# mmSir/SpatioTemporalEntropyModel

Hardware: AMD Instinct MI355X
Metric: frames/s (higher is better)
Workload: dtype f32; 1 GPU; configs[1]: SpatioTemporalPriorModel_Res(256,192) training step on mbt2018(192,192) latents, 16 septuplets x 7 frames x 256x256 per GPU, EMLoss, clip 1.0 + Adam 1e-4 / aux Adam 1e-3; per_gpu_batch=16, global_batch=16, parallelism=dp1, stream_priorities=latents=0,side=-1,compute=-1, stream_cu_masks=latents=block:160, plan_selectors=library defaults

## Files before the change

spatiotemporalentropymodel_amd/csrc/conv_f16x3.hip:

```cpp
#include <math.h>
#include <stdlib.h>

#include <type_traits>

#include "f16x3_tail.h"

namespace {

constexpr int XP = BN + 4;
constexpr int imax(int a, int b) { return a > b ? a : b; }
constexpr int lds_stages(int depth) { return depth == 3 ? 3 : 2; }
constexpr int lds_taps(int bm, int depth) { return imax(imax(lds_stages(depth) * NPL * (bm + BN) * 64, 6 * NPL * bm * 64 + NPL * BN * 64), bm * XP * 4); }
constexpr int lds_total(int bm, int depth) { return lds_taps(bm, depth) + 32 * 4; }

struct Fx3Phase {
    int ntaps, S;
    int dy0, dx0;
    int wofs;
    int cps, nsplit;
    int wsofs;
    int ooy, oox;
};

struct Fx3Args {
    const void *xp, *wp;
    const float *xq, *wq;
    float *yq;
    const float *bias, *beta;
    const void *gp;
    const float *gq;
    float *y;
    void *yp;
    int ldy;
    int B, H, W, C, N, OH, OW, stride, ntaps;
    int S;
    int xbytes, wbytes, gbytes;
    float beta_bound;
    int fuse;
    const float *z;
    int ldz, epi;
    float slope;
    float *ws;
    int *cnt;
    int nsplit, cps;
    int xpix;
    signed char dy[MAXTAP], dx[MAXTAP];
    int ptiles, btaps, OHf, OWf;
    Fx3Phase ph[4];
};

#define TAP_OFFSET(t) (tw_first + ((t) / tw_S) * tw_line + ((t) % tw_S) * tw_col)
#define TAP_WALK_NEXT()                                                                         \
    do {                                                                                        \
        const bool wrap_ = pf_t + 1 == tw_T, rowend_ = pf_ts + 1 == tw_S;                       \
        ++pf_q;                                                                                 \
        pf_to = wrap_ ? tw_first : pf_to + (rowend_ ? tw_line - (tw_S - 1) * tw_col : tw_col);  \
        pf_ts = (wrap_ || rowend_) ? 0 : pf_ts + 1;                                             \
        pf_t = wrap_ ? 0 : pf_t + 1;                                                            \
        pf_kc += wrap_ ? 1 : 0;                                                                 \
    } while (0)


__device__ inline int pi4(int x) { return (0x78 >> (2 * x)) & 3; }

typedef int rsrc4 __attribute__((ext_vector_type(4)));
__device__ inline rsrc4 dma_rsrc(const void *p, int bytes)
{
    const unsigned long long v = reinterpret_cast<unsigned long long>(p);
    return rsrc4{(int)(unsigned)v, (int)(unsigned)(v >> 32), bytes, 0x00020000};
}
__device__ inline void dma16(const rsrc4 r, unsigned lds_base, int voff, int soff)
{
    asm volatile("s_mov_b32 m0, %0\n\ts_nop 0\n\tbuffer_load_dwordx4 %1, %2, %3 offen lds" ::"s"(lds_base), "v"(voff), "s"(r), "s"(soff) : "memory");
}
#define DMA_WAIT_BARRIER(n) asm volatile("s_waitcnt vmcnt(%0)\n\ts_barrier" ::"n"(n) : "memory")
#define LDS_READS_DONE()                            \
    do {                                            \
        __builtin_amdgcn_sched_barrier(0);          \
        __builtin_amdgcn_s_waitcnt(0xC07F);         \
        __builtin_amdgcn_sched_barrier(0);          \
    } while (0)

template <int BM, int DEPTH, int MS>
__global__ __launch_bounds__(BM * 4) void conv_f16x3_kernel(const Fx3Args a)
{
    static_assert(DEPTH == 2 || DEPTH == 3, "two or three LDS stages");
    static_assert(MS == 32 || (MS == 16 && DEPTH == 3), "the 16-row MFMA shape exists for the three-stage loop");
    constexpr int NT = BM * 4;
    constexpr int A_PLANE = BM * 64, A_BUF = NPL * A_PLANE;
    constexpr int PL = NPL;
    constexpr int WPIECES = PL * BN * 4;
    static_assert(WPIECES % NT == 0, "every wavefront copies whole 1 KiB pieces of the weight chunk");
    constexpr int BP = WPIECES / NT;
    constexpr int NI = PL + BP;
    extern __shared__ __attribute__((aligned(16))) unsigned char smem[];
    constexpr int NST = lds_stages(DEPTH);
    unsigned char *As = smem;
    unsigned char *Bs = smem + NST * A_BUF;

    const int tid = threadIdx.x, lane = tid & 63, wave = tid >> 6;
    const int Mtot = a.B * a.OH * a.OW;
    int tile_m = blockIdx.x;
    {
        const int nb = gridDim.x, qq = nb >> 3, rr = nb & 7, xcd = tile_m & 7, idx = tile_m >> 3;
        if (nb >= 16) tile_m = (xcd < rr ? xcd * (qq + 1) : rr * (qq + 1) + (xcd - rr) * qq) + idx;
    }
    const int bm0 = tile_m * BM;
    const int nslab = a.C / KC, pixbytes = nslab * SLAB;

    const int srow = tid >> 2, scol = (tid & 3) ^ ((srow >> 2) & 3);
    int pb;
    unsigned pmask = 0;
    {
        const int m = bm0 + srow;
        const bool ok = m < Mtot;
        const int mm = ok ? m : 0;
        const int ohw = a.OH * a.OW, b = mm / ohw, rem = mm - b * ohw, qy = rem / a.OW, qx = rem - qy * a.OW;
        const int by = qy * a.stride, bx = qx * a.stride;
        pb = ((b * a.H + by) * a.W + bx) * pixbytes + scol * 16;
        for (int t = 0; t < a.ntaps; ++t) {
            const int iy = by + a.dy[t], ix = bx + a.dx[t];
            if (ok && iy >= 0 && iy < a.H && ix >= 0 && ix < a.W) pmask |= 1u << t;
        }
    }
    const int wv0 = tid * 16;
    const int nchunks = a.ntaps * nslab;
    const int q_last = nchunks - 1;
    __syncthreads();

    const rsrc4 rx = dma_rsrc(a.xp, a.xbytes), rw = dma_rsrc(a.wp, a.wbytes);
    const unsigned lds0 = (unsigned)(unsigned long long)(__attribute__((address_space(3))) unsigned char *)smem;
    const unsigned ldsw = __builtin_amdgcn_readfirstlane(lds0 + wave * 1024);
    auto dma_range = [&](int stage, int t, int tA, int kc, int q, int lo, int hi) {
        const int sA = kc * SLAB, sB = q * B_BUF;
        const int mk = __builtin_amdgcn_sbfe((int)pmask, (unsigned)t, 1u);
        const int off = ((pb + tA) & mk) | (OOR & ~mk);
        const unsigned la = ldsw + stage * A_BUF, lb = ldsw + NST * A_BUF + stage * B_BUF;
#pragma unroll
        for (int i = lo; i < hi; ++i) {
            if (i < PL)
                dma16(rx, la + i * A_PLANE, off + i * 64, sA);
            else
                dma16(rw, lb + (i - PL) * (NT * 16), wv0 + (i - PL) * (NT * 16), sB);
        }
    };
    auto dma = [&](int stage, int t, int tA, int kc, int q) { dma_range(stage, t, tA, kc, q, 0, NI); };

    const int wm0 = (wave >> 1) * 32, wn0 = (wave & 1) * 96;
    const int lr = lane & 31, lh = lane >> 5;
    const int sw = (lr >> 2) & 3;
    const int rdA = (wm0 + lr) * 64, rdB = (wn0 + lr) * 64;
    const int pk0 = ((0 + lh) ^ sw) << 4, pk1 = ((2 + lh) ^ sw) << 4;
    const int l16 = lane & 15, lq = lane >> 4;
    const int cm = 4 * pi4(l16 >> 2) + (l16 & 3), rq = 4 * pi4(lq);
    const int rdA16 = (wm0 + cm) * 64 + ((lq ^ pi4(l16 >> 2)) << 4), rdB16 = (wn0 + cm) * 64 + ((lq ^ pi4(l16 >> 2)) << 4);
    auto ROWL = [&](int r) { return MS == 32 ? wm0 + (r & 3) + 8 * (r >> 2) + 4 * lh : wm0 + ((r >> 2) & 1) * 16 + rq + (r & 3); };
    auto COLL = [&](int j, int r) { return MS == 32 ? wn0 + j * 32 + lr : wn0 + j * 32 + (r >> 3) * 16 + cm; };
    f32x16 acc[3];
#pragma unroll
    for (int j = 0; j < 3; ++j)
#pragma unroll
        for (int r = 0; r < 16; ++r) acc[j][r] = 0.f;

    int pf_q = 0, pf_t = 0, pf_kc = 0, pf_ts = 0, pf_to = 0;
    const int tw_T = a.ntaps, tw_S = a.S, tw_col = pixbytes, tw_line = a.W * pixbytes, tw_first = (a.dy[0] * a.W + a.dx[0]) * pixbytes;
    auto step = [&](int cur) {
        const unsigned char *Ab = As + cur * A_BUF + rdA, *Bb = Bs + cur * B_BUF + rdB;
        const int t = __builtin_amdgcn_readfirstlane(pf_t), kc = __builtin_amdgcn_readfirstlane(pf_kc), q = __builtin_amdgcn_readfirstlane(pf_q);
        const int to = __builtin_amdgcn_readfirstlane(pf_to);
        dma(cur ^ 1, t, to, kc, q);
#pragma unroll
        for (int ks = 0; ks < 2; ++ks) {
            const int pk = ks ? pk1 : pk0;
            h16x8 af[PL], bf[PL][3];
#pragma unroll
            for (int pl = 0; pl < PL; ++pl) af[pl] = *reinterpret_cast<const h16x8 *>(Ab + pl * A_PLANE + pk);
#pragma unroll
            for (int pl = 0; pl < PL; ++pl)
#pragma unroll
                for (int j = 0; j < 3; ++j) bf[pl][j] = *reinterpret_cast<const h16x8 *>(Bb + pl * B_PLANE + j * 32 * 64 + pk);
#pragma unroll
            for (int j = 0; j < 3; ++j) {
                acc[j] = STEM_MFMA16(af[1], bf[0][j], acc[j]);
                acc[j] = STEM_MFMA16(af[0], bf[1][j], acc[j]);
                acc[j] = STEM_MFMA16(af[0], bf[0][j], acc[j]);
            }
        }
        if (pf_q < q_last) TAP_WALK_NEXT();
        DMA_WAIT_BARRIER(0);
    };
// ... 72 lines not shown
    };
    auto mma18 = [&](h16x8 (&A)[2][PL], h16x8 (&B)[3][PL], int half, f32x4 (&d)[2][6]) {
#pragma unroll
        for (int prod = 0; prod < 3; ++prod)
#pragma unroll
            for (int n3 = 0; n3 < 3; ++n3)
#pragma unroll
                for (int mi = 0; mi < 2; ++mi)
                    d[mi][half * 3 + n3] = __builtin_amdgcn_mfma_f32_16x16x32_f16(A[mi][prod == 0 ? 1 : 0], B[n3][prod == 1 ? 1 : 0],
                                                                                   d[mi][half * 3 + n3], 0, 0, 0);
    };
    auto step3_16 = [&](int rd, int nx, h16x8 (&Acur)[2][PL], h16x8 (&Anext)[2][PL]) {
        const int t = __builtin_amdgcn_readfirstlane(pf_t), kc = __builtin_amdgcn_readfirstlane(pf_kc), q = __builtin_amdgcn_readfirstlane(pf_q);
        const int to = __builtin_amdgcn_readfirstlane(pf_to);
        lfragB16(Bs + rd * B_BUF, 1, gb1);
        mma18(Acur, gb0, 0, a16);
#pragma unroll
        for (int i = 0; i < 6; ++i) {
            __builtin_amdgcn_sched_group_barrier(0x008, 2, 0);
            __builtin_amdgcn_sched_group_barrier(0x100, 1, 0);
        }
        __builtin_amdgcn_sched_group_barrier(0x008, 6, 0);
        LDS_READS_DONE();
        DMA_WAIT_BARRIER(NI);
        auto ygroup = [&](auto group_tag) {
            constexpr int g = decltype(group_tag)::value;
            constexpr int r0 = g < 2 ? 3 * g : g < 4 ? 2 * g + 2 : 10, r1 = g < 1 ? 3 : g < 3 ? 2 * g + 4 : 10;
            constexpr int m0 = (g * 18 + 4) / 5, m1 = ((g + 1) * 18 + 4) / 5;
            dma_range(rd, t, to, kc, q, (g * NI + 4) / 5, ((g + 1) * NI + 4) / 5);
#pragma unroll
            for (int r = r0; r < r1; ++r) {
                if (r < 4)
                    Anext[r >> 1][r & 1] = *reinterpret_cast<const h16x8 *>(As + nx * A_BUF + rdA16 + (r >> 1) * 16 * 64 + (r & 1) * A_PLANE);
                else
                    gb0[(r - 4) >> 1][r & 1] = *reinterpret_cast<const h16x8 *>(Bs + nx * B_BUF + rdB16 + ((r - 4) >> 1) * 16 * 64 + (r & 1) * B_PLANE);
            }
#pragma unroll
            for (int m = m0; m < m1; ++m) {
                const int prod = m / 6, n3 = (m % 6) >> 1, mi = m & 1;
                a16[mi][3 + n3] = __builtin_amdgcn_mfma_f32_16x16x32_f16(Acur[mi][prod == 0 ? 1 : 0], gb1[n3][prod == 1 ? 1 : 0], a16[mi][3 + n3], 0, 0, 0);
            }
            if constexpr (r1 > r0) __builtin_amdgcn_sched_group_barrier(0x100, r1 - r0, 0);
            __builtin_amdgcn_sched_group_barrier(0x008, m1 - m0, 0);
        };
        ygroup(std::integral_constant<int, 0>{});
        ygroup(std::integral_constant<int, 1>{});
        ygroup(std::integral_constant<int, 2>{});
        ygroup(std::integral_constant<int, 3>{});
        ygroup(std::integral_constant<int, 4>{});
        LDS_READS_DONE();
        if (pf_q < q_last) TAP_WALK_NEXT();
    };

    auto chunk_of = [&](int q, int &t, int &kc) {
        q = q < q_last ? q : q_last;
        kc = q / a.ntaps;
        t = q - kc * a.ntaps;
        return q;
    };
    {
        int t, kc, q;
        constexpr int PRE = DEPTH == 3 ? 3 : 1;
#pragma unroll
        for (int c = 0; c < PRE; ++c) {
            q = chunk_of(c, t, kc);
            dma(c, t, TAP_OFFSET(t), kc, q);
        }
        pf_q = chunk_of(PRE, pf_t, pf_kc);
        pf_ts = pf_t % tw_S;
        pf_to = TAP_OFFSET(pf_t);
    }
    __shared__ float qred[16];
    const float fac = q_inv(a.xq) * q_inv(a.wq);
    float oscale = 1.f;
    if (a.yp) {
        const float xmax = q_amax(a.xq, qred), wmax = q_amax(a.wq, qred);
        float bm = 0.f, btm = 3.0e38f;
        for (int n = tid; n < a.N; n += NT) {
            if (a.bias) bm = fmaxf(bm, fabsf(a.bias[n]));
            if (a.fuse) {
                const float bb = fmaxf(a.beta[n], a.beta_bound);
                btm = fminf(btm, bb * bb - 1.4551915228366852e-11f);
            }
        }
        bm = block_max(bm, qred);
        float ob = (float)(a.C * a.ntaps) * xmax * wmax + bm;
        if (a.fuse) ob *= __builtin_amdgcn_rsqf(fmaxf(-block_max(-btm, qred), 1e-30f));
        const int oe = q_exp(ob);
        oscale = q_pow2(oe);
        if (blockIdx.x == 0 && tid == 0) a.yq[1] = q_pow2(-oe);
    }
    __syncthreads();
    DMA_WAIT_BARRIER(DEPTH == 3 ? 2 * NI : 0);
    if constexpr (MS == 16) {
        int rd = 0, nx = 1, wr = 2;
        lfragA16(As, ga[0]);
        lfragB16(Bs, 0, gb0);
        LDS_READS_DONE();
        int q = 0;
        for (; q + 1 < nchunks; q += 2) {
            step3_16(rd, nx, ga[0], ga[1]);
            step3_16(nx, wr, ga[1], ga[0]);
            const int o = rd;
            rd = wr; wr = nx; nx = o;
        }
        if (q < nchunks) step3_16(rd, nx, ga[0], ga[1]);
#pragma unroll
        for (int j = 0; j < 3; ++j)
#pragma unroll
            for (int r = 0; r < 16; ++r) acc[j][r] = a16[(r >> 2) & 1][2 * j + (r >> 3)][r & 3];
    } else if constexpr (DEPTH == 3) {
        int rd = 0, nx = 1, wr = 2;
        lfrag(0, pk0, f0a, f0b);
        LDS_READS_DONE();
        int q = 0;
        for (; q + 1 < nchunks; q += 2) {
#pragma unroll
            for (int s = 0; s < 2; ++s) {
                step3(rd, nx);
                const int o = rd;
                rd = nx; nx = wr; wr = o;
            }
        }
        if (q < nchunks) step3(rd, nx);
    } else {
        int q = 0;
        for (; q + 1 < nchunks; q += 2) {
#pragma unroll
            for (int s = 0; s < 2; ++s) step(s);
        }
        if (q < nchunks) step(0);
    }
    asm volatile("s_waitcnt vmcnt(0)" ::: "memory");
    __syncthreads();

    float *X2 = reinterpret_cast<float *>(smem);
    float omax = 0.f;
#pragma unroll
    for (int j = 0; j < 3; ++j) {
        float bias2[2];
#pragma unroll
        for (int h = 0; h < 2; ++h) {
            const int n = COLL(j, h * 8);
            bias2[h] = (a.bias && n < a.N) ? a.bias[n] : 0.f;
        }
#pragma unroll
        for (int r = 0; r < 16; ++r) acc[j][r] = acc[j][r] * fac + bias2[r >> 3];
// ... 432 lines not shown
    return conv2d_f16x3_launch(xp, xq, wp, bias, beta, gp, beta_min, 0, 0.f, y, ldy, yp, yq, B, H, W, C, N, R, S, stride, pad, stream);
}

STEM_EXPORT int stem_conv2d_f16x3_fwd_act(const void *xp, const float *xq, const void *wp, const float *bias, int act, float slope, float *y, int ldy,
                                           void *yp, float *yq, int B, int H, int W, int C, int N, int R, int S, int stride, int pad, void *stream)
{
    STEM_CHECK_ARG(act == 0 || act == 1, "stem_conv2d_f16x3_fwd_act: act is 0 (none) or 1 (leaky ReLU with `slope`)");
    STEM_CHECK_ARG(!act || fabsf(slope) <= 1.f, "stem_conv2d_f16x3_fwd_act: |slope| <= 1");
    return conv2d_f16x3_launch(xp, xq, wp, bias, nullptr, nullptr, 1e-6f, act, slope, y, ldy, yp, yq, B, H, W, C, N, R, S, stride, pad, stream);
}

static int conv2d_f16x3_launch(const void *xp, const float *xq, const void *wp, const float *bias, const float *beta, const void *gp,
                                float beta_min, int act, float slope, float *y, int ldy, void *yp, float *yq, int B, int H, int W, int C, int N,
                                int R, int S, int stride, int pad, void *stream)
{
    STEM_CHECK_ARG(xp && xq && wp && (y || yp) && (yq || !yp), "stem_conv2d_f16x3_fwd: null pointer (planes come with their scale records)");
    STEM_CHECK_ARG(B >= 1 && H >= 1 && W >= 1 && C >= 32 && C % 32 == 0 && N >= 1 && N <= BN && R >= 1 && S >= 1 && R * S <= MAXTAP &&
                   stride >= 1 && pad >= 0, "stem_conv2d_f16x3_fwd: C %% 32 == 0, N <= %d, R*S <= %d (C=%d N=%d R=%d S=%d)", BN, MAXTAP, C, N, R, S);
    STEM_CHECK_ARG(!yp || N % 32 == 0, "stem_conv2d_f16x3_fwd: planes output needs N %% 32 == 0 (N=%d)", N);
    STEM_CHECK_ARG(!y || ldy >= N, "stem_conv2d_f16x3_fwd: ldy < N");
    STEM_CHECK_ARG((beta == nullptr) == (gp == nullptr), "stem_conv2d_f16x3_fwd: beta and the packed gamma come together");
    const int OH = (H + 2 * pad - R) / stride + 1, OW = (W + 2 * pad - S) / stride + 1;
    STEM_CHECK_ARG(OH >= 1 && OW >= 1, "stem_conv2d_f16x3_fwd: empty output");
    const size_t xb = planes_payload((long)B * H * W, C), wb = w_image_bytes(C, R, S);
    STEM_CHECK_ARG(xb < 0x7FFFFF00ull && wb < 0x7FFFFF00ull && (size_t)B * OH * OW < 0x7FFFFFFFull,
                   "stem_conv2d_f16x3_fwd: operand views must stay below 2 GiB (split the batch)");
    Fx3Args a;
    memset(&a, 0, sizeof(a));
    a.xp = xp; a.wp = wp; a.bias = bias; a.beta = beta; a.gp = gp; a.y = y; a.yp = yp; a.ldy = ldy;
    if (gp) {
        const int cpad = cdiv(N, 32) * 32;
        a.gbytes = (int)w_image_bytes(cpad, 1, 1);
        a.gq = reinterpret_cast<const float *>(static_cast<const unsigned char *>(gp) + a.gbytes);
    }
    a.xq = xq; a.yq = yq; a.wq = reinterpret_cast<const float *>(static_cast<const unsigned char *>(wp) + wb);
    a.B = B; a.H = H; a.W = W; a.C = C; a.N = N; a.OH = OH; a.OW = OW; a.stride = stride; a.ntaps = R * S; a.S = S;
    a.xbytes = (int)xb; a.wbytes = (int)wb;
    a.fuse = gp ? 1 : 0;
    a.epi = act; a.slope = slope;
    a.beta_bound = (float)sqrt((double)beta_min + 1.4551915228366852e-11);
    for (int r = 0; r < R; ++r)
        for (int s = 0; s < S; ++s) {
            a.dy[r * S + s] = (signed char)(r - pad);
            a.dx[r * S + s] = (signed char)(s - pad);
        }
    static bool attr_done = false;
    if (!attr_done) {
        (void)hipFuncSetAttribute((const void *)conv_f16x3_kernel<128, 2, 32>, hipFuncAttributeMaxDynamicSharedMemorySize, lds_total(128, 2));
        (void)hipFuncSetAttribute((const void *)conv_f16x3_kernel<128, 3, 32>, hipFuncAttributeMaxDynamicSharedMemorySize, lds_total(128, 3));
        (void)hipFuncSetAttribute((const void *)conv_f16x3_kernel<128, 3, 16>, hipFuncAttributeMaxDynamicSharedMemorySize, lds_total(128, 3));
        (void)hipFuncSetAttribute((const void *)conv_f16x3_kernel<64, 2, 32>, hipFuncAttributeMaxDynamicSharedMemorySize, lds_total(64, 2));
        (void)hipFuncSetAttribute((const void *)conv_f16x3_kernel<64, 3, 32>, hipFuncAttributeMaxDynamicSharedMemorySize, lds_total(64, 3));
        (void)hipFuncSetAttribute((const void *)conv_f16x3_kernel<64, 3, 16>, hipFuncAttributeMaxDynamicSharedMemorySize, lds_total(64, 3));
        attr_done = true;
    }
    const int M = B * OH * OW;
    hipStream_t st = (hipStream_t)stream;
    const int tile = stem_tuning(STEM_TUNE_FX3_TILE);
    const bool small = tile ? tile == 64 : cdiv(M, 128) < 128;
    const int dsel = stem_tuning(STEM_TUNE_FX3_DEPTH);
    const int depth = dsel ? dsel : (small ? 2 : 3);
    const int msel = stem_tuning(STEM_TUNE_FX3_MFMA);
    const bool m16 = depth == 3 && (msel ? msel == 16 : !small);
    stem_ran_note(STEM_RAN_FX3_COL_TILE, small ? 64 : 128);
    stem_ran_note(STEM_RAN_FX3_COL_DEPTH, depth == 3 ? 3 : 2);
    stem_ran_note(STEM_RAN_FX3_COL_MFMA, m16 ? 16 : 32);
    if (small && m16)
        hipLaunchKernelGGL((conv_f16x3_kernel<64, 3, 16>), dim3(cdiv(M, 64)), dim3(256), lds_total(64, 3), st, a);
    else if (small && depth == 3)
        hipLaunchKernelGGL((conv_f16x3_kernel<64, 3, 32>), dim3(cdiv(M, 64)), dim3(256), lds_total(64, 3), st, a);
    else if (small)
        hipLaunchKernelGGL((conv_f16x3_kernel<64, 2, 32>), dim3(cdiv(M, 64)), dim3(256), lds_total(64, 2), st, a);
    else if (m16)
        hipLaunchKernelGGL((conv_f16x3_kernel<128, 3, 16>), dim3(cdiv(M, 128)), dim3(512), lds_total(128, 3), st, a);
    else if (depth == 3)
        hipLaunchKernelGGL((conv_f16x3_kernel<128, 3, 32>), dim3(cdiv(M, 128)), dim3(512), lds_total(128, 3), st, a);
    else
        hipLaunchKernelGGL((conv_f16x3_kernel<128, 2, 32>), dim3(cdiv(M, 128)), dim3(512), lds_total(128, 2), st, a);
    STEM_LAUNCH_CHECK("stem_conv2d_f16x3_fwd");
    return 0;
}

namespace {
constexpr size_t kGenCntBytes = 64 * 1024;

int gen_split(int tiles, int nchunks)
{
    const int forced = stem_tuning(STEM_TUNE_FX3_SPLIT);
    if (forced > 0) return forced < nchunks ? forced : nchunks;
    if (nchunks <= 40 && tiles >= 128) return 1;
    int best = 1;
    double best_cost = 1e30;
    for (int s = 1; s <= 16 && s * 8 <= nchunks; ++s) {
        const int cps = cdiv(nchunks, s), ns = cdiv(nchunks, cps), rounds = cdiv(tiles * ns, 256);
        const double cost = rounds * (cps + 6.0) * (rounds == 1 ? 1.67 : 1.0) + (ns > 1 ? 0.3 * ns : 0.0);
        if (cost < best_cost - 1e-9) {
            best_cost = cost;
            best = ns;
        }
    }
    return best;
}

int gen_bm(int M, int ntn, int nchunks)
{
    const int forced = stem_tuning(STEM_TUNE_FX3_GEN_TILE);
    if (forced) return forced;
    (void)nchunks;
    return cdiv(M, 128) * ntn >= 64 ? 128 : 64;
}
}

STEM_EXPORT size_t stem_conv2d_f16x3_gen_workspace_bytes(int B, int H, int W, int C, int N, int R, int S, int stride, int pad, int taps)
{
    const int OH = (H + 2 * pad - R) / stride + 1, OW = (W + 2 * pad - S) / stride + 1;
    if (OH < 1 || OW < 1 || C % 32) return 0;
    const int M = B * OH * OW, nchunks = (C / 32) * (taps > 0 ? taps : R * S), tiles = cdiv(M, gen_bm(M, cdiv(N, GBN), nchunks)) * cdiv(N, GBN);
    int s = gen_split(tiles, nchunks);
    if (stem_fx3_img_eligible(B, H, W, N, R, S, stride, pad)) {
        const int si = stem_fx3_img_split(stem_fx3_img_tiles(B, H, W, N), nchunks);
// ... 198 lines not shown
```

spatiotemporalentropymodel_amd/csrc/pack.hip:

```cpp
#include <stdarg.h>

#include "stem_common.h"

static thread_local char g_err[512] = "";
void stem_set_error(const char *fmt, ...)
{
    va_list ap;
    va_start(ap, fmt);
    vsnprintf(g_err, sizeof(g_err), fmt, ap);
    va_end(ap);
}
STEM_EXPORT const char *stem_last_error(void) { return g_err; }
STEM_EXPORT int stem_abi_version(void) { return 5; }

static int g_tuning[STEM_TUNE_COUNT] = {0};
static const char *const kTuningNames[STEM_TUNE_COUNT] = {"fx3_tile", "fx3_split", "wg3_split", "arp_workers", "fx3_depth", "fx3_gen_tile", "fx3_mfma", "fx3_gen_mfma", "fx3_gen_img", "fx3_img_w", "wg3_row", "wg3_minch", "tconv_cps", "arp_giveup_at", "unpack_mb", "igemm_cfg", "igemm_fuse_cfg", "igemm_split", "wgrad_cfg"};
static int g_ran[STEM_RAN_COUNT] = {0};
static const char *const kRanNames[STEM_RAN_COUNT] = {"igemm_ran_cfg", "igemm_ran_split", "wgrad_ran_cfg", "fx3_ran_form", "fx3_ran_split", "fx3_ran_mfma", "wg3_ran_form", "wg3_ran_taps", "wg3_ran_split", "fx3_col_ran_tile", "fx3_col_ran_depth", "fx3_col_ran_mfma", "tconv_ran_tile", "tconv_ran_cps", "tconv_ran_split0", "tconv_ran_split1", "tconv_ran_split2", "tconv_ran_split3"};
void stem_ran_note(int id, int value) { g_ran[id] = value; }
int stem_tuning(int id) { return g_tuning[id]; }
STEM_EXPORT int stem_tuning_set(const char *name, int value)
{
    STEM_CHECK_ARG(name && value >= 0, "stem_tuning_set: null name or negative value");
    for (int i = 0; i < STEM_RAN_COUNT; ++i)
        STEM_CHECK_ARG(strcmp(name, kRanNames[i]), "stem_tuning_set: %s is get-only (the plan of the most recent launch)", name);
    for (int i = 0; i < STEM_TUNE_COUNT; ++i)
        if (!strcmp(name, kTuningNames[i])) {
            STEM_CHECK_ARG(i != STEM_TUNE_FX3_TILE || value == 0 || value == 64 || value == 128, "stem_tuning_set: fx3_tile is 0 (automatic), 64 or 128");
            STEM_CHECK_ARG(i != STEM_TUNE_FX3_GEN_TILE || value == 0 || value == 64 || value == 128, "stem_tuning_set: fx3_gen_tile is 0 (automatic), 64 or 128");
            STEM_CHECK_ARG(i != STEM_TUNE_FX3_DEPTH || value == 0 || value == 2 || value == 3, "stem_tuning_set: fx3_depth is 0 (automatic), 2 or 3 (LDS stages of the split-operand main loops)");
            STEM_CHECK_ARG(i != STEM_TUNE_FX3_GEN_MFMA || value == 0 || value == 16 || value == 32, "stem_tuning_set: fx3_gen_mfma is 0 (automatic), 16 or 32 (rows of the general kernel's MFMA shape)");
            STEM_CHECK_ARG(i != STEM_TUNE_UNPACK_MB || value == 0 || (value % 32 == 0 && value >= 32 && value <= 192), "stem_tuning_set: unpack_mb is 0 (automatic) or a multiple of 32 up to 192");
            STEM_CHECK_ARG(i != STEM_TUNE_FX3_MFMA || value == 0 || value == 16 || value == 32, "stem_tuning_set: fx3_mfma is 0 (automatic), 16 or 32 (rows of the MFMA shape)");
            STEM_CHECK_ARG(i != STEM_TUNE_IGEMM_CFG || value <= 6, "stem_tuning_set: igemm_cfg is 0 (automatic) or 1..6 (tile 128x128, 64x192, 128x64, 64x64, 128x192 / 8 waves, 128x128 / 8 waves)");
            STEM_CHECK_ARG(i != STEM_TUNE_IGEMM_FUSE_CFG || value == 0 || value == 2 || value == 5, "stem_tuning_set: igemm_fuse_cfg is 0 (automatic), 2 or 5 (the 192-wide tiles 64x192 and 128x192 of the fused-GDN kernels)");
            STEM_CHECK_ARG(i != STEM_TUNE_WGRAD_CFG || value <= 5, "stem_tuning_set: wgrad_cfg is 0 (automatic) or 1..5 (tile 128x128, 128x64, 64x128, 64x64, 128x128 / 8 waves)");
            g_tuning[i] = value;
            return 0;
        }
    stem_set_error("stem_tuning_set: unknown selector '%s' (fx3_tile, fx3_split, wg3_split, arp_workers, fx3_depth, fx3_gen_tile, fx3_mfma, fx3_gen_mfma, fx3_gen_img, fx3_img_w, wg3_row, wg3_minch, tconv_cps, arp_giveup_at, unpack_mb, igemm_cfg, igemm_fuse_cfg, igemm_split, wgrad_cfg)", name);
    return -1;
}
STEM_EXPORT int stem_tuning_get(const char *name)
{
    for (int i = 0; name && i < STEM_TUNE_COUNT; ++i)
        if (!strcmp(name, kTuningNames[i])) return g_tuning[i];
    for (int i = 0; name && i < STEM_RAN_COUNT; ++i)
        if (!strcmp(name, kRanNames[i])) return g_ran[i];
    return -1;
}

namespace {

__global__ __launch_bounds__(256) void pack_kernel(float *w, float *out, int A, int Bd, int T, long sa, long sb,
                                                   int R, int S, int masked)
{
    extern __shared__ float tile[];
    const int a = blockIdx.x;
    const int n = Bd * T;
    for (int i = threadIdx.x; i < n; i += 256) {
        const int b = i / T, t = i - b * T;
        float v = w[a * sa + b * sb + t];
        if (masked & 3) {
            const int r = t / S, s = t - r * S;
            if (r > R / 2 || (r == R / 2 && s >= S / 2 + ((masked >> 2) & 1))) {
                v = 0.f;
                if ((masked & 3) == 2) w[a * sa + b * sb + t] = 0.f;
            }
        }
        tile[i] = v;
    }
    __syncthreads();
    for (int i = threadIdx.x; i < n; i += 256) {
        const int t = i / Bd, b = i - t * Bd;
        out[((size_t)t * A + a) * Bd + b] = tile[b * T + t];
    }
}

constexpr int MAXD = 32;
struct PackD {
    float *w;
    float *out;
    int A, Bd, T, R, S, masked, block0;
    long sa, sb;
};
struct PackTable {
    PackD d[MAXD];
    int n;
};
__global__ __launch_bounds__(256) void pack_multi_kernel(const PackTable tb)
{
    extern __shared__ float tile[];
    int i = 0;
// ... 391 lines not shown
```

spatiotemporalentropymodel_amd/csrc/stem_common.h:

```cpp
#pragma once
#include <hip/hip_runtime.h>
#include <stdint.h>
#include <stdio.h>
#include <string.h>

#include "../../include/stem_hip.h"

#define STEM_EXPORT extern "C" __attribute__((visibility("default")))

void stem_set_error(const char *fmt, ...);

#define STEM_CHECK_ARG(cond, ...)        \
    do {                                 \
        if (!(cond)) {                   \
            stem_set_error(__VA_ARGS__); \
            return -1;                   \
        }                                \
    } while (0)

#define STEM_LAUNCH_CHECK(name)                                                         \
    do {                                                                                \
        hipError_t e_ = hipGetLastError();                                              \
        if (e_ != hipSuccess) {                                                         \
            stem_set_error("%s: launch failed: %s", name, hipGetErrorString(e_));       \
            return -2;                                                                  \
        }                                                                               \
    } while (0)

typedef float f32x4 __attribute__((ext_vector_type(4)));
typedef float f32x16 __attribute__((ext_vector_type(16)));

static inline int cdiv(int a, int b) { return (a + b - 1) / b; }
static inline size_t cdivz(size_t a, size_t b) { return (a + b - 1) / b; }

enum { STEM_TUNE_FX3_TILE = 0, STEM_TUNE_FX3_SPLIT, STEM_TUNE_WG3_SPLIT, STEM_TUNE_ARP_WORKERS, STEM_TUNE_FX3_DEPTH, STEM_TUNE_FX3_GEN_TILE, STEM_TUNE_FX3_MFMA, STEM_TUNE_FX3_GEN_MFMA, STEM_TUNE_FX3_GEN_IMG, STEM_TUNE_FX3_IMG_W, STEM_TUNE_WG3_ROW, STEM_TUNE_WG3_MINCH, STEM_TUNE_TCONV_CPS, STEM_TUNE_ARP_GIVEUP_AT, STEM_TUNE_UNPACK_MB, STEM_TUNE_IGEMM_CFG, STEM_TUNE_IGEMM_FUSE_CFG, STEM_TUNE_IGEMM_SPLIT, STEM_TUNE_WGRAD_CFG, STEM_TUNE_COUNT };
enum { STEM_RAN_IGEMM_CFG = 0, STEM_RAN_IGEMM_SPLIT, STEM_RAN_WGRAD_CFG, STEM_RAN_FX3_FORM, STEM_RAN_FX3_SPLIT, STEM_RAN_FX3_MFMA, STEM_RAN_WG3_FORM, STEM_RAN_WG3_TAPS, STEM_RAN_WG3_SPLIT, STEM_RAN_FX3_COL_TILE, STEM_RAN_FX3_COL_DEPTH, STEM_RAN_FX3_COL_MFMA, STEM_RAN_TCONV_TILE, STEM_RAN_TCONV_CPS, STEM_RAN_TCONV_SPLIT0, STEM_RAN_TCONV_SPLIT1, STEM_RAN_TCONV_SPLIT2, STEM_RAN_TCONV_SPLIT3, STEM_RAN_COUNT };
void stem_ran_note(int id, int value);
int stem_tuning(int id);
bool stem_fx3_img_eligible(int B, int H, int W, int N, int R, int S, int stride, int pad);
int stem_fx3_img_tiles(int B, int H, int W, int N);
int stem_fx3_img_split(int tiles, int nchunks);
int stem_fx3_img_launch(const void *xp, const float *xq, int xpix, int xbytes, const void *wp, const float *wq, int wbytes, const float *bias, int epi,
                        float slope, const float *z, int ldz, float *y, int ldy, void *yp, float *yq, int B, int H, int W, int C, int N, int KS,
                        int T, int split, float *ws, int *cnt, void *stream);

#define STEM_ADAM_CHUNK 4096

typedef _Float16 hp_t;
typedef hp_t hp8 __attribute__((ext_vector_type(8)));
#define STEM_MFMA16(a, b, c) __builtin_amdgcn_mfma_f32_32x32x16_f16(a, b, c, 0, 0, 0)

constexpr int QREC_HDR = 16;
#ifdef __HIPCC__
__device__ inline int q_nslots(const float *q) { return reinterpret_cast<const int *>(q)[0]; }
__device__ inline float q_inv(const float *q) { return q[1]; }
__device__ inline void q_header(float *q, int n)
{
    reinterpret_cast<int *>(q)[0] = n;
#pragma unroll
    for (int i = 2; i < QREC_HDR; ++i) q[i] = 0.f;
}
__device__ inline int q_exp(float bound)
{
    const unsigned b = __float_as_uint(bound) & 0x7FFFFFFFu;
    int eb = (int)(b >> 23) - 127;
    if (b == 0u || eb == 128) return 0;
    if (eb < -126) eb = -126;
    const int e = 14 - eb;
    return e > 126 ? 126 : e;
}
__device__ inline float q_pow2(int e) { return __uint_as_float((unsigned)(e + 127) << 23); }
__device__ inline float wave_max(float v)
{
#pragma unroll
    for (int o = 32; o; o >>= 1) v = fmaxf(v, __shfl_xor(v, o));
    return v;
}
template <int NT = 0>
__device__ inline float block_max(float v, float *red)
{
    v = wave_max(v);
    __syncthreads();
    if ((threadIdx.x & 63) == 0) red[threadIdx.x >> 6] = v;
    __syncthreads();
    float m = red[0];
    for (int w = 1; w < (NT ? NT >> 6 : (int)(blockDim.x >> 6)); ++w) m = fmaxf(m, red[w]);
    return m;
}
__device__ inline float q_amax(const float *q, float *red)
// ... 45 lines not shown
```

Measured before the change: 10270 frames/s.

## Add filter-row form of the f16x3 5x5 stride-2 conv staging input rows in LDS

Adds a new kernel variant for 5x5 stride-2 pad-2 convolutions. For each filter row and channel slab it loads one strip of input image rows into LDS, split into even and odd columns, and reads all five horizontal taps from that strip. The existing form DMAs a separate A tile for every tap. The new form is meant to cut global/L2 traffic and DMA issue count for the input operand. In exchange it adds more LDS usage, a new fixed pipeline schedule and indexing complexity. It is enabled by default for eligible shapes with the 128-row, 16-wide MFMA configuration.

```diff
diff --git a/spatiotemporalentropymodel_amd/csrc/conv_f16x3.hip b/spatiotemporalentropymodel_amd/csrc/conv_f16x3.hip
--- a/spatiotemporalentropymodel_amd/csrc/conv_f16x3.hip
+++ b/spatiotemporalentropymodel_amd/csrc/conv_f16x3.hip
@@ -3,6 +3,7 @@
 
 #include <type_traits>
 
+#include "f16x3_rows.h"
 #include "f16x3_tail.h"
 
 namespace {
@@ -12,6 +13,14 @@
 constexpr int lds_stages(int depth) { return depth == 3 ? 3 : 2; }
 constexpr int lds_taps(int bm, int depth) { return imax(imax(lds_stages(depth) * NPL * (bm + BN) * 64, 6 * NPL * bm * 64 + NPL * BN * 64), bm * XP * 4); }
 constexpr int lds_total(int bm, int depth) { return lds_taps(bm, depth) + 32 * 4; }
+constexpr int ROWS_I_PLANE = FX3_ROWS_IROWS * 64, ROWS_I_BUF = NPL * ROWS_I_PLANE;
+constexpr int lds_rows_main() { return 2 * ROWS_I_BUF + 3 * B_BUF; }
+constexpr int lds_rows_total() { return imax(lds_rows_main(), lds_taps(FX3_ROWS_BM, 3)) + 32 * 4; }
+constexpr bool FX3_ROWS_DEFAULT = true;
+static_assert(ROWS_I_BUF == FX3_ROWS_PIECES * 1024, "an image is FX3_ROWS_PIECES LDS-DMA pieces");
+static_assert(6 * NPL * FX3_ROWS_BM * 64 + NPL * BN * 64 <= lds_rows_main() && FX3_ROWS_BM * XP * 4 <= lds_rows_main(),
+              "the fused GDN and the planes pass fit into the row form's ring");
+static_assert(lds_rows_total() + 16 * 4 <= 160 * 1024, "row form: images + weight stages + the reduction scratch within 160 KiB of LDS");
 
 struct Fx3Phase {
     int ntaps, S;
@@ -81,11 +90,12 @@
         __builtin_amdgcn_sched_barrier(0);          \
     } while (0)
 
-template <int BM, int DEPTH, int MS>
+template <int BM, int DEPTH, int MS, bool ROWS = false>
 __global__ __launch_bounds__(BM * 4) void conv_f16x3_kernel(const Fx3Args a)
 {
     static_assert(DEPTH == 2 || DEPTH == 3, "two or three LDS stages");
     static_assert(MS == 32 || (MS == 16 && DEPTH == 3), "the 16-row MFMA shape exists for the three-stage loop");
+    static_assert(!ROWS || (BM == FX3_ROWS_BM && DEPTH == 3 && MS == 16), "the filter-row form exists for <128, 3, 16>");
     constexpr int NT = BM * 4;
     constexpr int A_PLANE = BM * 64, A_BUF = NPL * A_PLANE;
     constexpr int PL = NPL;
@@ -95,8 +105,9 @@
     constexpr int NI = PL + BP;
     extern __shared__ __attribute__((aligned(16))) unsigned char smem[];
     constexpr int NST = lds_stages(DEPTH);
+    constexpr int A_RING = ROWS ? 2 * ROWS_I_BUF : NST * A_BUF;
     unsigned char *As = smem;
-    unsigned char *Bs = smem + NST * A_BUF;
+    unsigned char *Bs = smem + A_RING;
 
     const int tid = threadIdx.x, lane = tid & 63, wave = tid >> 6;
     const int Mtot = a.B * a.OH * a.OW;
@@ -135,7 +146,7 @@
         const int sA = kc * SLAB, sB = q * B_BUF;
         const int mk = __builtin_amdgcn_sbfe((int)pmask, (unsigned)t, 1u);
         const int off = ((pb + tA) & mk) | (OOR & ~mk);
-        const unsigned la = ldsw + stage * A_BUF, lb = ldsw + NST * A_BUF + stage * B_BUF;
+        const unsigned la = ldsw + stage * A_BUF, lb = ldsw + A_RING + stage * B_BUF;
 #pragma unroll
         for (int i = lo; i < hi; ++i) {
             if (i < PL)
@@ -314,13 +325,109 @@
         if (pf_q < q_last) TAP_WALK_NEXT();
     };
 
+    int ioff[5] = {0, 0, 0, 0, 0};
+    unsigned vmask = 0;
+    int arow[2] = {0, 0};
+    const int TW = fx3_rows_tw(a.OW);
+    if constexpr (ROWS) {
+        const int g0 = bm0 / a.OW, qx0 = bm0 - g0 * a.OW, seg = fx3_rows_seg(TW), nseg = BM / TW;
+#pragma unroll
+        for (int j = 0; j < 5; ++j) {
+            const int P = 8 * j + wave, pl = P / (FX3_ROWS_PIECES / 2), row = 16 * (P % (FX3_ROWS_PIECES / 2)) + (lane >> 2);
+            const int r = row / seg, rem = row - r * seg, par = rem >= TW + 2 ? 1 : 0, idx = rem - par * (TW + 2);
+            const int g = g0 + r, ix = fx3_rows_column(qx0, par, idx);
+            const bool ok = r < nseg && g < a.B * a.OH && ix >= 0 && ix < a.W;
+            const int gg = ok ? g : 0, b = gg / a.OH, qy = gg - b * a.OH, iy0 = 2 * qy - 2;
+            ioff[j] = ok ? ((b * a.H + iy0) * a.W + ix) * pixbytes + pl * 64 + (((lane & 3) ^ fx3_rows_swz(row)) << 4) : 0;
+#pragma unroll
+            for (int dy = 0; dy < 5; ++dy)
+                if (ok && iy0 + dy >= 0 && iy0 + dy < a.H) vmask |= 1u << (5 * j + dy);
+        }
+#pragma unroll
+        for (int mi = 0; mi < 2; ++mi) arow[mi] = fx3_rows_frag_row(TW, wm0 + 16 * mi, -2, lane);
+    }
+    auto rows_img = [&](int stage, int j, int kc, int dy) {
+        const int mk = __builtin_amdgcn_sbfe((int)(vmask >> (5 * j + dy)), 0u, 1u);
+        dma16(rx, ldsw + stage * ROWS_I_BUF + j * 8192, ((ioff[j] + dy * tw_line) & mk) | (OOR & ~mk), kc * SLAB);
+    };
+    auto rows_wgt = [&](int stage, int q, int u) {
+        dma16(rw, ldsw + A_RING + stage * B_BUF + u * (NT * 16), wv0 + u * (NT * 16), q * B_BUF);
+    };
+    auto rows_aaddr = [&](int mi, int ti) { return fx3_rows_row_addr(arow[mi] + (ti & 1) * (TW + 2) + (ti >> 1), lane); };
+    auto rstep = [&](auto itag, auto ptag, int rd, int nx, int q, int kc1, int dy1, int kc2, int dy2) {
+        constexpr int I = decltype(itag)::value, PAR = decltype(ptag)::value;
+        constexpr int NDMA = I == 4 ? 5 : I == 3 ? 3 : 4;
+        constexpr int VM = I == 0 ? 5 : I == 4 ? 3 : 4;
+        constexpr int IST = I < 4 ? PAR : PAR ^ 1, TN = (I + 1) % 5;
+        h16x8 (&Acur)[2][PL] = ga[(PAR + I) & 1];
+        h16x8 (&Anext)[2][PL] = ga[(PAR + I + 1) & 1];
+        const int qw = q + 3 < q_last ? q + 3 : q_last;
+        const unsigned char *An[2] = {As + IST * ROWS_I_BUF + rows_aaddr(0, TN), As + IST * ROWS_I_BUF + rows_aaddr(1, TN)};
+        lfragB16(Bs + rd * B_BUF, 1, gb1);
+        mma18(Acur, gb0, 0, a16);
+#pragma unroll
+        for (int i = 0; i < 6; ++i) {
+            __builtin_amdgcn_sched_group_barrier(0x008, 2, 0);
+            __builtin_amdgcn_sched_group_barrier(0x100, 1, 0);
+        }
+        __builtin_amdgcn_sched_group_barrier(0x008, 6, 0);
+        LDS_READS_DONE();
+        DMA_WAIT_BARRIER(VM);
+        auto ygroup = [&](auto group_tag) {
+            constexpr int g = decltype(group_tag)::value;
+            constexpr int r0 = g < 2 ? 3 * g : g < 4 ? 2 * g + 2 : 10, r1 = g < 1 ? 3 : g < 3 ? 2 * g + 4 : 10;
+            constexpr int m0 = (g * 18 + 4) / 5, m1 = ((g + 1) * 18 + 4) / 5;
+#pragma unroll
+            for (int k = (g * NDMA + 4) / 5; k < ((g + 1) * NDMA + 4) / 5; ++k) {
+                if (k < BP)
+                    rows_wgt(rd, qw, k);
+                else if (I < 3)
+                    rows_img(PAR ^ 1, I + 2, kc1, dy1);
+                else
+                    rows_img(PAR, k - BP, kc2, dy2);
+            }
+#pragma unroll
+            for (int r = r0; r < r1; ++r) {
+                if (r < 4)
+                    Anext[r >> 1][r & 1] = *reinterpret_cast<const h16x8 *>(An[r >> 1] + (r & 1) * ROWS_I_PLANE);
+                else
+                    gb0[(r - 4) >> 1][r & 1] = *reinterpret_cast<const h16x8 *>(Bs + nx * B_BUF + rdB16 + ((r - 4) >> 1) * 16 * 64 + (r & 1) * B_PLANE);
+            }
+#pragma unroll
+            for (int m = m0; m < m1; ++m) {
+                const int prod = m / 6, n3 = (m % 6) >> 1, mi = m & 1;
+                a16[mi][3 + n3] = __builtin_amdgcn_mfma_f32_16x16x32_f16(Acur[mi][prod == 0 ? 1 : 0], gb1[n3][prod == 1 ? 1 : 0], a16[mi][3 + n3], 0, 0, 0);
+            }
+            if constexpr (r1 > r0) __builtin_amdgcn_sched_group_barrier(0x100, r1 - r0, 0);
+            __builtin_amdgcn_sched_group_barrier(0x008, m1 - m0, 0);
+        };
+        ygroup(std::integral_constant<int, 0>{});
+        ygroup(std::integral_constant<int, 1>{});
+        ygroup(std::integral_constant<int, 2>{});
+        ygroup(std::integral_constant<int, 3>{});
+        ygroup(std::integral_constant<int, 4>{});
+        LDS_READS_DONE();
+    };
+
     auto chunk_of = [&](int q, int &t, int &kc) {
         q = q < q_last ? q : q_last;
         kc = q / a.ntaps;
         t = q - kc * a.ntaps;
         return q;
     };
-    {
+    (void)rows_img; (void)rows_wgt; (void)rows_aaddr;
+    if constexpr (ROWS) {
+#pragma unroll
+        for (int j = 0; j < 5; ++j) rows_img(0, j, 0, 0);
+#pragma unroll
+        for (int c = 0; c < 2; ++c)
+#pragma unroll
+            for (int u = 0; u < BP; ++u) rows_wgt(c, c, u);
+        rows_img(1, 0, 0, 1);
+        rows_img(1, 1, 0, 1);
+#pragma unroll
+        for (int u = 0; u < BP; ++u) rows_wgt(2, 2, u);
+    } else {
         int t, kc, q;
         constexpr int PRE = DEPTH == 3 ? 3 : 1;
 #pragma unroll
@@ -353,8 +460,41 @@
         if (blockIdx.x == 0 && tid == 0) a.yq[1] = q_pow2(-oe);
     }
     __syncthreads();
-    DMA_WAIT_BARRIER(DEPTH == 3 ? 2 * NI : 0);
-    if constexpr (MS == 16) {
+    DMA_WAIT_BARRIER(ROWS ? 2 * BP + 2 : DEPTH == 3 ? 2 * NI : 0);
+    if constexpr (ROWS) {
+        int rd = 0, nx = 1, wr = 2;
+        const int nrows = 5 * nslab;
+#pragma unroll
+        for (int mi = 0; mi < 2; ++mi)
+#pragma unroll
+            for (int pl = 0; pl < PL; ++pl) ga[0][mi][pl] = *reinterpret_cast<const h16x8 *>(As + rows_aaddr(mi, 0) + pl * ROWS_I_PLANE);
+        lfragB16(Bs, 0, gb0);
+        LDS_READS_DONE();
+        auto frow = [&](auto ptag, int f) {
+            const int f1 = f + 1 < nrows ? f + 1 : nrows - 1, f2 = f + 2 < nrows ? f + 2 : nrows - 1;
+            const int kc1 = f1 / 5, dy1 = f1 - 5 * kc1, kc2 = f2 / 5, dy2 = f2 - 5 * kc2;
+            auto one = [&](auto itag) {
+                rstep(itag, ptag, rd, nx, 5 * f + decltype(itag)::value, kc1, dy1, kc2, dy2);
+                const int o = rd;
+                rd = nx; nx = wr; wr = o;
+            };
+            one(std::integral_constant<int, 0>{});
+            one(std::integral_constant<int, 1>{});
+            one(std::integral_constant<int, 2>{});
+            one(std::integral_constant<int, 3>{});
+            one(std::integral_constant<int, 4>{});
+        };
+        int f = 0;
+        for (; f + 1 < nrows; f += 2) {
+            frow(std::integral_constant<int, 0>{}, f);
+            frow(std::integral_constant<int, 1>{}, f + 1);
+        }
+        if (f < nrows) frow(std::integral_constant<int, 0>{}, f);
+#pragma unroll
+        for (int j = 0; j < 3; ++j)
+#pragma unroll
+            for (int r = 0; r < 16; ++r) acc[j][r] = a16[(r >> 2) & 1][2 * j + (r >> 3)][r & 3];
+    } else if constexpr (MS == 16) {
         int rd = 0, nx = 1, wr = 2;
         lfragA16(As, ga[0]);
         lfragB16(Bs, 0, gb0);
@@ -893,6 +1033,7 @@
         (void)hipFuncSetAttribute((const void *)conv_f16x3_kernel<64, 2, 32>, hipFuncAttributeMaxDynamicSharedMemorySize, lds_total(64, 2));
         (void)hipFuncSetAttribute((const void *)conv_f16x3_kernel<64, 3, 32>, hipFuncAttributeMaxDynamicSharedMemorySize, lds_total(64, 3));
         (void)hipFuncSetAttribute((const void *)conv_f16x3_kernel<64, 3, 16>, hipFuncAttributeMaxDynamicSharedMemorySize, lds_total(64, 3));
+        (void)hipFuncSetAttribute((const void *)conv_f16x3_kernel<128, 3, 16, true>, hipFuncAttributeMaxDynamicSharedMemorySize, lds_rows_total());
         attr_done = true;
     }
     const int M = B * OH * OW;
@@ -906,7 +1047,12 @@
     stem_ran_note(STEM_RAN_FX3_COL_TILE, small ? 64 : 128);
     stem_ran_note(STEM_RAN_FX3_COL_DEPTH, depth == 3 ? 3 : 2);
     stem_ran_note(STEM_RAN_FX3_COL_MFMA, m16 ? 16 : 32);
-    if (small && m16)
+    const int rsel = stem_tuning(STEM_TUNE_FX3_ROWS);
+    const bool rows = !small && m16 && fx3_rows_shape_ok(R, S, stride, pad, OW) && (rsel ? rsel == 2 : FX3_ROWS_DEFAULT);
+    stem_ran_note(STEM_RAN_FX3_COL_ROWS, rows ? 2 : 1);
+    if (rows)
+        hipLaunchKernelGGL((conv_f16x3_kernel<128, 3, 16, true>), dim3(cdiv(M, 128)), dim3(512), lds_rows_total(), st, a);
+    else if (small && m16)
         hipLaunchKernelGGL((conv_f16x3_kernel<64, 3, 16>), dim3(cdiv(M, 64)), dim3(256), lds_total(64, 3), st, a);
     else if (small && depth == 3)
         hipLaunchKernelGGL((conv_f16x3_kernel<64, 3, 32>), dim3(cdiv(M, 64)), dim3(256), lds_total(64, 3), st, a);
diff --git a/spatiotemporalentropymodel_amd/csrc/f16x3_rows.h b/spatiotemporalentropymodel_amd/csrc/f16x3_rows.h
--- /dev/null
+++ b/spatiotemporalentropymodel_amd/csrc/f16x3_rows.h
@@ -0,0 +1,32 @@
+#pragma once
+
+#if defined(__HIPCC__)
+#define FX3_ROWS_FN __host__ __device__ inline
+#else
+#define FX3_ROWS_FN inline
+#endif
+
+constexpr int FX3_ROWS_BM = 128;
+constexpr int FX3_ROWS_PIECES = 40;
+constexpr int FX3_ROWS_IROWS = FX3_ROWS_PIECES * 16 / 2;
+
+FX3_ROWS_FN bool fx3_rows_shape_ok(int R, int S, int stride, int pad, int OW)
+{
+    return R == 5 && S == 5 && stride == 2 && pad == 2 && OW % 16 == 0 && (FX3_ROWS_BM % OW == 0 || OW % FX3_ROWS_BM == 0);
+}
+FX3_ROWS_FN int fx3_rows_tw(int OW) { return OW < FX3_ROWS_BM ? OW : FX3_ROWS_BM; }
+FX3_ROWS_FN int fx3_rows_seg(int TW) { return 2 * TW + 3; }
+FX3_ROWS_FN int fx3_rows_swz(int row) { return ((row >> 2) & 1) << 1; }
+FX3_ROWS_FN int fx3_rows_tap_parity(int dx) { return dx & 1; }
+FX3_ROWS_FN int fx3_rows_tap_shift(int dx) { return (dx - (dx & 1)) / 2 + 1; }
+FX3_ROWS_FN int fx3_rows_row(int TW, int r, int parity, int idx) { return r * fx3_rows_seg(TW) + parity * (TW + 2) + idx; }
+FX3_ROWS_FN int fx3_rows_column(int qx0, int parity, int idx) { return parity ? 2 * (qx0 + idx) - 1 : 2 * (qx0 + idx - 1); }
+FX3_ROWS_FN int fx3_rows_pi4(int x) { return (0x78 >> (2 * x)) & 3; }
+FX3_ROWS_FN int fx3_rows_lane_pixel(int lane) { return 4 * fx3_rows_pi4((lane & 15) >> 2) + (lane & 3); }
+FX3_ROWS_FN int fx3_rows_frag_row(int TW, int pix0, int dx, int lane)
+{
+    const int r = pix0 / TW, lx = pix0 - r * TW + fx3_rows_lane_pixel(lane);
+    return fx3_rows_row(TW, r, fx3_rows_tap_parity(dx), lx + fx3_rows_tap_shift(dx));
+}
+FX3_ROWS_FN int fx3_rows_row_addr(int row, int lane) { return row * 64 + (((lane >> 4) ^ fx3_rows_swz(row)) << 4); }
+FX3_ROWS_FN int fx3_rows_frag_addr(int TW, int pix0, int dx, int lane) { return fx3_rows_row_addr(fx3_rows_frag_row(TW, pix0, dx, lane), lane); }
diff --git a/spatiotemporalentropymodel_amd/csrc/pack.hip b/spatiotemporalentropymodel_amd/csrc/pack.hip
--- a/spatiotemporalentropymodel_amd/csrc/pack.hip
+++ b/spatiotemporalentropymodel_amd/csrc/pack.hip
@@ -14,9 +14,9 @@
 STEM_EXPORT int stem_abi_version(void) { return 5; }
 
 static int g_tuning[STEM_TUNE_COUNT] = {0};
-static const char *const kTuningNames[STEM_TUNE_COUNT] = {"fx3_tile", "fx3_split", "wg3_split", "arp_workers", "fx3_depth", "fx3_gen_tile", "fx3_mfma", "fx3_gen_mfma", "fx3_gen_img", "fx3_img_w", "wg3_row", "wg3_minch", "tconv_cps", "arp_giveup_at", "unpack_mb", "igemm_cfg", "igemm_fuse_cfg", "igemm_split", "wgrad_cfg"};
+static const char *const kTuningNames[STEM_TUNE_COUNT] = {"fx3_tile", "fx3_split", "wg3_split", "arp_workers", "fx3_depth", "fx3_gen_tile", "fx3_mfma", "fx3_gen_mfma", "fx3_gen_img", "fx3_img_w", "wg3_row", "wg3_minch", "tconv_cps", "arp_giveup_at", "unpack_mb", "igemm_cfg", "igemm_fuse_cfg", "igemm_split", "wgrad_cfg", "fx3_rows"};
 static int g_ran[STEM_RAN_COUNT] = {0};
-static const char *const kRanNames[STEM_RAN_COUNT] = {"igemm_ran_cfg", "igemm_ran_split", "wgrad_ran_cfg", "fx3_ran_form", "fx3_ran_split", "fx3_ran_mfma", "wg3_ran_form", "wg3_ran_taps", "wg3_ran_split", "fx3_col_ran_tile", "fx3_col_ran_depth", "fx3_col_ran_mfma", "tconv_ran_tile", "tconv_ran_cps", "tconv_ran_split0", "tconv_ran_split1", "tconv_ran_split2", "tconv_ran_split3"};
+static const char *const kRanNames[STEM_RAN_COUNT] = {"igemm_ran_cfg", "igemm_ran_split", "wgrad_ran_cfg", "fx3_ran_form", "fx3_ran_split", "fx3_ran_mfma", "wg3_ran_form", "wg3_ran_taps", "wg3_ran_split", "fx3_col_ran_tile", "fx3_col_ran_depth", "fx3_col_ran_mfma", "tconv_ran_tile", "tconv_ran_cps", "tconv_ran_split0", "tconv_ran_split1", "tconv_ran_split2", "tconv_ran_split3", "fx3_col_ran_rows"};
 void stem_ran_note(int id, int value) { g_ran[id] = value; }
 int stem_tuning(int id) { return g_tuning[id]; }
 STEM_EXPORT int stem_tuning_set(const char *name, int value)
@@ -35,10 +35,11 @@
             STEM_CHECK_ARG(i != STEM_TUNE_IGEMM_CFG || value <= 6, "stem_tuning_set: igemm_cfg is 0 (automatic) or 1..6 (tile 128x128, 64x192, 128x64, 64x64, 128x192 / 8 waves, 128x128 / 8 waves)");
             STEM_CHECK_ARG(i != STEM_TUNE_IGEMM_FUSE_CFG || value == 0 || value == 2 || value == 5, "stem_tuning_set: igemm_fuse_cfg is 0 (automatic), 2 or 5 (the 192-wide tiles 64x192 and 128x192 of the fused-GDN kernels)");
             STEM_CHECK_ARG(i != STEM_TUNE_WGRAD_CFG || value <= 5, "stem_tuning_set: wgrad_cfg is 0 (automatic) or 1..5 (tile 128x128, 128x64, 64x128, 64x64, 128x128 / 8 waves)");
+            STEM_CHECK_ARG(i != STEM_TUNE_FX3_ROWS || value <= 2, "stem_tuning_set: fx3_rows is 0 (automatic), 1 (per-tap form) or 2 (filter-row form wherever eligible)");
             g_tuning[i] = value;
             return 0;
         }
-    stem_set_error("stem_tuning_set: unknown selector '%s' (fx3_tile, fx3_split, wg3_split, arp_workers, fx3_depth, fx3_gen_tile, fx3_mfma, fx3_gen_mfma, fx3_gen_img, fx3_img_w, wg3_row, wg3_minch, tconv_cps, arp_giveup_at, unpack_mb, igemm_cfg, igemm_fuse_cfg, igemm_split, wgrad_cfg)", name);
+    stem_set_error("stem_tuning_set: unknown selector '%s' (fx3_tile, fx3_split, wg3_split, arp_workers, fx3_depth, fx3_gen_tile, fx3_mfma, fx3_gen_mfma, fx3_gen_img, fx3_img_w, wg3_row, wg3_minch, tconv_cps, arp_giveup_at, unpack_mb, igemm_cfg, igemm_fuse_cfg, igemm_split, wgrad_cfg, fx3_rows)", name);
     return -1;
 }
 STEM_EXPORT int stem_tuning_get(const char *name)
diff --git a/spatiotemporalentropymodel_amd/csrc/stem_common.h b/spatiotemporalentropymodel_amd/csrc/stem_common.h
--- a/spatiotemporalentropymodel_amd/csrc/stem_common.h
+++ b/spatiotemporalentropymodel_amd/csrc/stem_common.h
@@ -33,8 +33,8 @@
 static inline int cdiv(int a, int b) { return (a + b - 1) / b; }
 static inline size_t cdivz(size_t a, size_t b) { return (a + b - 1) / b; }
 
-enum { STEM_TUNE_FX3_TILE = 0, STEM_TUNE_FX3_SPLIT, STEM_TUNE_WG3_SPLIT, STEM_TUNE_ARP_WORKERS, STEM_TUNE_FX3_DEPTH, STEM_TUNE_FX3_GEN_TILE, STEM_TUNE_FX3_MFMA, STEM_TUNE_FX3_GEN_MFMA, STEM_TUNE_FX3_GEN_IMG, STEM_TUNE_FX3_IMG_W, STEM_TUNE_WG3_ROW, STEM_TUNE_WG3_MINCH, STEM_TUNE_TCONV_CPS, STEM_TUNE_ARP_GIVEUP_AT, STEM_TUNE_UNPACK_MB, STEM_TUNE_IGEMM_CFG, STEM_TUNE_IGEMM_FUSE_CFG, STEM_TUNE_IGEMM_SPLIT, STEM_TUNE_WGRAD_CFG, STEM_TUNE_COUNT };
-enum { STEM_RAN_IGEMM_CFG = 0, STEM_RAN_IGEMM_SPLIT, STEM_RAN_WGRAD_CFG, STEM_RAN_FX3_FORM, STEM_RAN_FX3_SPLIT, STEM_RAN_FX3_MFMA, STEM_RAN_WG3_FORM, STEM_RAN_WG3_TAPS, STEM_RAN_WG3_SPLIT, STEM_RAN_FX3_COL_TILE, STEM_RAN_FX3_COL_DEPTH, STEM_RAN_FX3_COL_MFMA, STEM_RAN_TCONV_TILE, STEM_RAN_TCONV_CPS, STEM_RAN_TCONV_SPLIT0, STEM_RAN_TCONV_SPLIT1, STEM_RAN_TCONV_SPLIT2, STEM_RAN_TCONV_SPLIT3, STEM_RAN_COUNT };
+enum { STEM_TUNE_FX3_TILE = 0, STEM_TUNE_FX3_SPLIT, STEM_TUNE_WG3_SPLIT, STEM_TUNE_ARP_WORKERS, STEM_TUNE_FX3_DEPTH, STEM_TUNE_FX3_GEN_TILE, STEM_TUNE_FX3_MFMA, STEM_TUNE_FX3_GEN_MFMA, STEM_TUNE_FX3_GEN_IMG, STEM_TUNE_FX3_IMG_W, STEM_TUNE_WG3_ROW, STEM_TUNE_WG3_MINCH, STEM_TUNE_TCONV_CPS, STEM_TUNE_ARP_GIVEUP_AT, STEM_TUNE_UNPACK_MB, STEM_TUNE_IGEMM_CFG, STEM_TUNE_IGEMM_FUSE_CFG, STEM_TUNE_IGEMM_SPLIT, STEM_TUNE_WGRAD_CFG, STEM_TUNE_FX3_ROWS, STEM_TUNE_COUNT };
+enum { STEM_RAN_IGEMM_CFG = 0, STEM_RAN_IGEMM_SPLIT, STEM_RAN_WGRAD_CFG, STEM_RAN_FX3_FORM, STEM_RAN_FX3_SPLIT, STEM_RAN_FX3_MFMA, STEM_RAN_WG3_FORM, STEM_RAN_WG3_TAPS, STEM_RAN_WG3_SPLIT, STEM_RAN_FX3_COL_TILE, STEM_RAN_FX3_COL_DEPTH, STEM_RAN_FX3_COL_MFMA, STEM_RAN_TCONV_TILE, STEM_RAN_TCONV_CPS, STEM_RAN_TCONV_SPLIT0, STEM_RAN_TCONV_SPLIT1, STEM_RAN_TCONV_SPLIT2, STEM_RAN_TCONV_SPLIT3, STEM_RAN_FX3_COL_ROWS, STEM_RAN_COUNT };
 void stem_ran_note(int id, int value);
 int stem_tuning(int id);
 bool stem_fx3_img_eligible(int B, int H, int W, int N, int R, int S, int stride, int pad);
```

Result: no change. 10320 frames/s (median of 6 runs) (+0.5%).
